# crisbodnar/text-to-image

Hardware: AMD Instinct MI355X
Metric: images/sec (G+D step) at 64x64 batch=64 (higher is better)
Workload: dtype f32; 1 GPU; wgancls 64x64 batch=64/GPU fp32, synthetic images + random 1024-d text embeddings, D step (+kt) then G step, Adam(b1=0,b2=0.9); global_batch=64, parallelism=dp1, launch=hipGraph replay (1 graph/iteration)

## Files before the change

### text-to-image_amd/csrc/t2i_bgemm.hip

```cpp
#include <hip/hip_runtime.h>
#include <stdint.h>

#include <type_traits>

#include "t2i_internal.h"

namespace t2i {

typedef float f32x16 __attribute__((ext_vector_type(16)));
typedef unsigned int u32x4 __attribute__((ext_vector_type(4)));

namespace {
constexpr int BK = 32;
constexpr int KSTRIDE = BK + 4;
constexpr unsigned OOB = 0xFFFFFFF0u;

template <int LAY, int WM, int WN, int NW = 4>
struct BSmem {
  static constexpr bool A_KIN = LAY != 2, B_KIN = LAY == 1;
  static constexpr int BM = 32 * (NW / 2) * WM, BN = 64 * WN;
  static constexpr int A_ELEMS = A_KIN ? BM * KSTRIDE : BK * BM;
  static constexpr int B_ELEMS = B_KIN ? BN * KSTRIDE : BK * BN;
  static constexpr int BYTES = 2 * (A_ELEMS + B_ELEMS) * 4;
};
// ... 29 lines not shown
  const int n_items = (runlen - slot + nslot - 1) / nslot;
  const int tiles = p.tiles_m * p.tiles_n;

  auto coords = [&](int w, int& bz, int& bm, int& bn) __attribute__((always_inline)) {
    bz = w / tiles;
    const int t = w - bz * tiles;
    const int g = p.group_n, per_group = g * p.tiles_m;
    const int grp = t / per_group, rr = t - grp * per_group, n0 = grp * g;
    const int width = min(g, p.tiles_n - n0);
    const int tm = rr / width;
    bm = tm * BM;
    bn = (n0 + rr - tm * width) * BN;
  };

  const int kq = tid & 7, r0 = tid >> 3;
  const int a_c4 = tid % A_C4, a_kr = tid / A_C4, b_c4 = tid % B_C4, b_kr = tid / B_C4;
  __amdgpu_buffer_rsrc_t ra, rb;
  int a_off[A_LD], b_off[B_LD];
  bool a_ok[A_LD], b_ok[B_LD];
  int l_item = -1, l_t = 0;

  auto next_item = [&]() __attribute__((always_inline)) {
    ++l_item;
    l_t = 0;
    if (l_item >= n_items) {
#pragma unroll
      for (int i = 0; i < A_LD; ++i) a_ok[i] = false;
#pragma unroll
      for (int i = 0; i < B_LD; ++i) b_ok[i] = false;
      return;
    }
    int bz, bm, bn;
    coords(run0 + slot + l_item * nslot, bz, bm, bn);
    ra = __builtin_amdgcn_make_buffer_rsrc(const_cast<float*>(p.a + (int64_t)bz * p.sa), (short)0, (int)p.a_bytes, 0x00020000);
    rb = __builtin_amdgcn_make_buffer_rsrc(const_cast<float*>(p.b + (int64_t)bz * p.sb), (short)0, (int)p.b_bytes, 0x00020000);
#pragma unroll
    for (int i = 0; i < A_LD; ++i) {
      if (A_KIN) {
        const int m = bm + r0 + RPP * i;
        a_ok[i] = m < p.M;
        a_off[i] = m * p.K + kq * 4;
      } else {
        const int m = bm + a_c4 * 4;
        a_ok[i] = m < p.M;
        a_off[i] = (a_kr + A_KR * i) * p.M + m;
      }
    }
#pragma unroll
    for (int i = 0; i < B_LD; ++i) {
      if (B_KIN) {
        const int n = bn + r0 + RPP * i;
        b_ok[i] = n < p.N;
        b_off[i] = n * p.K + kq * 4;
      } else {
        const int n = bn + b_c4 * 4;
        b_ok[i] = n < p.N;
        b_off[i] = (b_kr + B_KR * i) * p.N + n;
      }
    }
  };

  float4 areg[A_LD], breg[B_LD];
  auto load_into = [&](float4* ar, float4* br) __attribute__((always_inline)) {
    const int k0 = l_t * BK;
    ++l_t;
#pragma unroll
    for (int i = 0; i < A_LD; ++i) {
      if (A_KIN) ar[i] = bl4(ra, a_off[i] + k0, a_ok[i] & (k0 + kq * 4 < p.K));
// ... 674 lines not shown
```

### text-to-image_amd/csrc/t2i_capi.hip

```cpp
#include <hip/hip_runtime.h>
#include <atomic>
#include <initializer_list>
#include <stdarg.h>
#include <stdio.h>
#include <stdlib.h>
#include <string.h>

#include "t2i_internal.h"

namespace t2i {

static thread_local char g_err[512] = "";

void set_error(const char* fmt, ...) {
  va_list ap;
  va_start(ap, fmt);
  vsnprintf(g_err, sizeof(g_err), fmt, ap);
  va_end(ap);
}

size_t col_reduce_ws(int64_t rows, int C);
hipError_t col_reduce_launch(const void*, const void*, const float*, int64_t, int, float*, float*, int, void*, hipStream_t, bool in_bf16 = false);
hipError_t bn_stats_launch(const void*, int64_t, int, float*, float*, const float*, const float*, float, float, float*, float*, float*,
                           float*, float*, float*, void*, hipStream_t, bool x_bf16 = false);
// ... 165 lines not shown
    v.bgemm = env_int("T2I_BGEMM", 1);
    v.bgemm_tile = env_int("T2I_BGEMM_TILE", 0);
    v.bgemm_big_items = env_int("T2I_BGEMM_BIG_ITEMS", 2048);
    v.dma_ovh = env_int("T2I_DMA_OVH", 120);
    v.dma_split_us = env_int("T2I_DMA_SPLIT_US", 29);
    v.tile8_eff = env_int("T2I_TILE8_EFF", 0);
    v.colred_wgs = env_int("T2I_COLRED_WGS", 768);
    v.wino_fuse = env_int("T2I_WINO_FUSE", 1);
    v.wino_fuse_items = env_int("T2I_WINO_FUSE_ITEMS", 512);
    v.wino_fuse_xf = env_int("T2I_WINO_FUSE_XF", 1);
    v.bn_fuse = env_int("T2I_BN_FUSE", 1);
    v.colred_cap = env_int("T2I_COLRED_CAP", 192);
    v.bf16_waves = env_int("T2I_BF16_WAVES", 8);
    v.bf16_pair_tiles = env_int("T2I_BF16_PAIR_TILES", 0);
    v.pair_reduce = env_int("T2I_PAIR_REDUCE", 1);
    v.h_stats = env_int("T2I_H_STATS", 0);
    v.pair_cus = env_int("T2I_PAIR_CUS", 128);
    v.pair_max_px = env_int("T2I_PAIR_MAX_PX", 49152);
    v.pair = env_int("T2I_PAIR", 1);
    v.vec_epi = env_int("T2I_VEC_EPI", 1);
    v.batch_lin = env_int("T2I_BATCH_LIN", 1);
    v.no_ut = env_int("T2I_NO_UT", 0);
    v.no_thin = env_int("T2I_NO_THIN", 0);
    v.winograd = env_int("T2I_WINOGRAD", 1);
    v.winograd_minc = env_int("T2I_WINOGRAD_MINC", 128);
    v.winograd_maxhw = env_int("T2I_WINOGRAD_MAXHW", 1024);
    v.winograd_minwork = env_int("T2I_WINOGRAD_MINWORK", 50000000);
    v.winograd_k4s2 = env_int("T2I_WINOGRAD_K4S2", 1);
    v.winograd_k4s2_minc = env_int("T2I_WINOGRAD_K4S2_MINC", 128);
    v.winograd_k4s2_bwd_minc = env_int("T2I_WINOGRAD_K4S2_BWD_MINC", 128);
    v.winograd_k4s2_bwdf = env_int("T2I_WINOGRAD_K4S2_BWDF", 1);
    v.winograd_k4s2_minwork = env_int("T2I_WINOGRAD_K4S2_MINWORK", 160000000);
    v.winograd_k4s2_minitems = env_int("T2I_WINOGRAD_K4S2_MINITEMS", 400);
    v.adam_blocks = env_int("T2I_ADAM_BLOCKS", 2048);
    v.cache_refresh = env_int("T2I_CACHE_REFRESH", 0);
    v.thin_parts = env_int("T2I_THIN_PARTS", 2);
    v.bf16_operands = env_int("T2I_BF16_OPERANDS", 1);
    v.max_chain = env_int("T2I_MAX_CHAIN", 8192);
    const char* sc = getenv("T2I_SPLIT_COST");
    v.split_cost = (sc && *sc) ? atof(sc) : 4.0;
    return v;
  }();
  return t;
}

const Tuning& tuning() { return tuning_mut(); }

static Plan make_plan(int64_t M, int64_t N, int64_t K, int nphase, size_t out_elems, int split_cap = 32, int math = 0, bool batched = false,
                      int bk = 32, int m_unit = 0,
                      bool dma = false,
                      int cus = 256) {
  static const int cand[5][2] = {{2, 2}, {2, 1}, {1, 2}, {1, 1}, {4, 2}};
  static const double rel_eff_f32[4] = {1.0, 0.93, 0.93, 0.94};
  static const double rel_eff_bf16[4] = {1.0, 0.74, 0.74, 0.55};
  static const int max_resident_f32[4] = {2, 3, 3, 4};
  static const int max_resident_bf16[4] = {3, 4, 4, 4};
  static const double share_eff_f32[5] = {0.0, 0.80, 0.95, 1.0, 1.0};
  static const double share_eff_bf16[5] = {0.0, 0.62, 0.86, 1.0, 1.0};
  const double rel_eff_dma[5] = {1.0, 0.82, 0.83, 0.64, tuning().tile8_eff * 0.01};
  static const int max_resident_dma[5] = {3, 3, 3, 6, 1};
  static const double share_eff_dma[7] = {0.0, 0.75, 1.0, 1.0, 1.0, 1.0, 1.0};
  const bool hft = math && m_unit > 0 && (m_unit % 128) == 0 && tuning().bf16_dma;
  const double hft_boost = hft ? tuning().hft_boost * 0.01 : 1.0;
  const double* rel_eff = dma ? rel_eff_dma : (math ? rel_eff_bf16 : rel_eff_f32);
  const int* max_resident = dma ? max_resident_dma : (math ? max_resident_bf16 : max_resident_f32);
  const double* share_eff = dma ? share_eff_dma : (math ? share_eff_bf16 : share_eff_f32);
// ... 287 lines not shown
    if (tuning().debug_plan) fprintf(stderr, "[t2i stage] cast_bf16 x (filter gradient): B=%d %dx%dx%d->%d k%d s%d\n", d->B, d->H, d->W, d->Cin, d->Cout, d->KH, d->SH);
    rc = check(cast_bf16_launch(x, nx, base, stream), what);
    if (rc != T2I_OK) return rc;
    x_h = base;
  }
  if (!dy_h || !aligned16(dy_h)) {
    if (tuning().debug_plan) fprintf(stderr, "[t2i stage] cast_bf16 dy (filter gradient): B=%d %dx%dx%d->%d k%d s%d\n", d->B, d->H, d->W, d->Cin, d->Cout, d->KH, d->SH);
    rc = check(cast_bf16_launch(dy, ny, base + off_y, stream), what);
    if (rc != T2I_OK) return rc;
    dy_h = base + off_y;
  }
  p.a = reinterpret_cast<const float*>(x_h); p.b = reinterpret_cast<const float*>(dy_h);
  p.a_bytes = (uint32_t)(nx * 2); p.b_bytes = (uint32_t)(ny * 2);
  p.tiles_m = pl.tiles_m; p.tiles_n = pl.tiles_n; p.group_n = 1;
  p.splitk = pl.splitk; p.k_per_split = pl.k_per_split;
  p.out_elems = out_elems;
  p.bias = nullptr; p.act = T2I_ACT_NONE; p.alpha = 0.f;
  if (pl.splitk > 1) { p.c = reinterpret_cast<float*>(base + off_s); p.accumulate = 0; }
  else { p.c = dw; p.accumulate = accumulate; }
  if (defer) {
    defer->set = true; defer->mode = MODE_BWD_FILTER; defer->wmt = pl.wmt; defer->wnt = pl.wnt; defer->p = p;
    defer->slabs = reinterpret_cast<const float*>(base + off_s); defer->bias = nullptr; defer->act = T2I_ACT_NONE; defer->alpha = 0.f; defer->out = dw;
    defer->accumulate = accumulate; defer->out_h = nullptr; defer->out_h_written = nullptr;
    return T2I_OK;
  }
  rc = check(igemm_h_filter_launch(p, pl.wmt, pl.wnt, stream), what);
  if (rc != T2I_OK) return rc;
  if (pl.splitk > 1)
    rc = check(splitk_reduce_launch(reinterpret_cast<const float*>(base + off_s), pl.splitk, out_elems, nullptr, p.N, T2I_ACT_NONE, 0.f, dw,
                                    accumulate, stream), what);
  return rc;
}

int run_batched_gemm(const t2i_conv_desc& gd, int gmode, int nbatch, const float* a, const float* b, float* c, int64_t sa, int64_t sb,
                     int64_t sc, hipStream_t stream, const char* what) {
  {
    const int M = gmode == MODE_BWD_FILTER ? gd.Cin : gd.B;
    const int N = gmode == MODE_BWD_DATA ? gd.Cin : gd.Cout;
    const int K = gmode == MODE_BWD_FILTER ? gd.B : (gmode == MODE_BWD_DATA ? gd.Cout : gd.Cin);
    const int ntiles = (K + 31) / 32;
    const int64_t a_elems = (int64_t)gd.B * (gmode == MODE_BWD_DATA ? gd.Cout : gd.Cin);
    const int64_t b_elems = gmode == MODE_BWD_FILTER ? (int64_t)gd.B * gd.Cout : (int64_t)gd.Cin * gd.Cout;
    if (tuning().bgemm && gd.math != T2I_MATH_BF16 && !tuning().force_tile && (ntiles & 1) == 0 && M % 4 == 0 && N % 4 == 0 && K % 4 == 0 &&
        aligned16(a) && aligned16(b) && sa % 4 == 0 && sb % 4 == 0 && a_elems < (1LL << 30) && b_elems < (1LL << 30)) {
      BgemmParams q;
      memset(&q, 0, sizeof(q));
      q.a = a; q.b = b; q.c = c;
      q.M = M; q.N = N; q.K = K;
      int wm = 1, wn = 1;
      {
        auto items_of = [&](int a_, int b_) { return (int64_t)nbatch * ((M + 64 * a_ - 1) / (64 * a_)) * ((N + 64 * b_ - 1) / (64 * b_)); };
        const int ft = tuning().bgemm_tile;
        const int64_t big = tuning().bgemm_big_items;
        if (ft == 22 || ft == 21 || ft == 12 || ft == 11) { wm = ft / 10; wn = ft % 10; }
        else if (ft == 41 && M >= 128) { wm = 4; wn = 1; }
        else if (M >= 128 && N >= 128 && items_of(2, 2) >= big) { wm = 2; wn = 2; }
        else if (M >= 128 && items_of(2, 1) >= big) { wm = 2; wn = 1; }
        else if (N >= 128 && items_of(1, 2) >= big) { wm = 1; wn = 2; }
      }
      const int bm_rows = wm == 4 ? 128 : 64 * wm;
      q.tiles_m = (M + bm_rows - 1) / bm_rows; q.tiles_n = (N + 64 * wn - 1) / (64 * wn);
      { const int g = tuning().group_n; q.group_n = q.tiles_n < g ? q.tiles_n : g; if (q.group_n < 1) q.group_n = 1; }
      q.ntiles = ntiles;
      const int64_t items = (int64_t)nbatch * q.tiles_m * q.tiles_n;
      if (items < (1LL << 30)) {
        q.items = (int32_t)items;
        q.sa = sa; q.sb = sb; q.sc = sc;
        q.a_bytes = (uint32_t)(a_elems * 4); q.b_bytes = (uint32_t)(b_elems * 4);
        if (tuning().debug_plan)
          fprintf(stderr, "[t2i plan] batched x%d M=%d N=%d K=%d mode %d -> persistent %dx%d, %lld items\n", nbatch, M, N, K, gmode, bm_rows, 64 * wn, (long long)items);
        return check(bgemm_launch(gmode == MODE_FWD ? 0 : (gmode == MODE_BWD_DATA ? 1 : 2), wm, wn, q, stream), what);
      }
    }
  }
  IgemmParams p;
  fill_common(p, &gd);
  p.a = a; p.b = b;
  if (gmode == MODE_BWD_FILTER) {
    p.a_bytes = (uint32_t)((size_t)gd.B * gd.Cin * 4);
    p.b_bytes = (uint32_t)((size_t)gd.B * gd.Cout * 4);
    p.M = gd.Cin; p.N = gd.Cout; p.K = gd.B;
    p.div_c.set(gd.Cin);
    p.walk_db = 32; p.walk_doh = 0;
    p.nbatch = nbatch; p.batch_a = sa; p.batch_b = sb; p.batch_c = sc; p.batch_lin = tuning().batch_lin;
    Plan pl = make_plan(p.M, p.N, p.K, nbatch, (size_t)p.M * p.N, 1, gd.math, true);
    p.tiles_m = pl.tiles_m; p.tiles_n = pl.tiles_n;
    { const int g = tuning().group_n; p.group_n = pl.tiles_n < g ? pl.tiles_n : g; if (p.group_n < 1) p.group_n = 1; }
    p.splitk = 1; p.k_per_split = pl.k_per_split;
    p.out_elems = (size_t)p.M * p.N;
    p.c = c; p.bias = nullptr; p.act = T2I_ACT_NONE; p.alpha = 0.f; p.accumulate = 0;
    const bool vec = (gd.Cin % 4 == 0) && (gd.Cout % 4 == 0) && aligned16(a) && aligned16(b);
    return check(igemm_launch(MODE_BWD_FILTER, p, pl.wmt, pl.wnt, vec ? 2 : 0, stream), what);
  }
  const bool bwd = gmode == MODE_BWD_DATA;
  const int K = bwd ? gd.Cout : gd.Cin, N = bwd ? gd.Cin : gd.Cout;
  p.a_bytes = (uint32_t)((size_t)gd.B * K * 4);
  p.b_bytes = (uint32_t)((size_t)gd.Cin * gd.Cout * 4);
  p.M = gd.B; p.N = N; p.K = K;
  if (bwd) {
    const int kmax = fill_phases(p);
    p.K = kmax;
    p.div_c.set(gd.Cout);
  } else {
    p.div_c.set(gd.Cin);
  }
  p.nbatch = nbatch; p.batch_a = sa; p.batch_b = sb; p.batch_c = sc; p.batch_lin = tuning().batch_lin;
  Plan pl = make_plan(p.M, p.N, p.K, nbatch, (size_t)p.M * p.N, 1, gd.math, true);
// ... 1151 lines not shown
  if (!w || !g || !v || !slot_end_dev || !slot_mult_dev) { set_error("t2i_adam_tf_slots: bad argument (w, g, v or a slot table is NULL)"); return T2I_ERR_INVALID; }
  if (n <= 0 || (n & 3)) { set_error("t2i_adam_tf_slots: n = %lld must be a positive multiple of 4", (long long)n); return T2I_ERR_INVALID; }
  if (n_slots < 1 || n_slots > T2I_ADAM_MAX_SLOTS) {
    set_error("t2i_adam_tf_slots: n_slots = %d is outside [1, %d]", (int)n_slots, (int)T2I_ADAM_MAX_SLOTS);
    return T2I_ERR_INVALID;
  }
  if (!adam_args_ok(a, ADAM_MOMENT | ADAM_ALIGNED)) return T2I_ERR_INVALID;
  if (reinterpret_cast<uintptr_t>(slot_end_dev) & 7) { set_error("t2i_adam_tf_slots: slot_end_dev must be 8-byte aligned"); return T2I_ERR_INVALID; }
  if (!adam_args_ok(a, ADAM_APART)) return T2I_ERR_INVALID;
  for (const float* o : {(const float*)w, g, (const float*)m, (const float*)v, (const float*)ema})
    if (ranges_overlap(slot_end_dev, (uintptr_t)n_slots * 8, o, (uintptr_t)n * 4) || ranges_overlap(slot_mult_dev, (uintptr_t)n_slots * 8, o, (uintptr_t)n * 4)) {
      set_error("t2i_adam_tf_slots: a slot table overlaps an arena");
      return T2I_ERR_INVALID;
    }
  if (!adam_args_ok(a, ADAM_DECAY)) return T2I_ERR_INVALID;
  return adam_update(a, slot_end_dev, slot_mult_dev, (int)n_slots, lr_t, lr_t_dev, beta2, eps, grad_scale, stream);
}

long long t2i_stat(const char* key) {
  if (key && !strcmp(key, "pair_fused")) return g_stat_pair_fused.load();
  return -1;
}

int t2i_tuning_set(const char* key, double value) {
  if (!key) { set_error("t2i_tuning_set: null key"); return T2I_ERR_INVALID; }
  Tuning& t = tuning_mut();
  struct { const char* name; int* field; } ints[] = {
      {"force_tile", &t.force_tile}, {"force_splitk", &t.force_splitk}, {"debug_plan", &t.debug_plan}, {"group_n", &t.group_n},
      {"no_ut", &t.no_ut}, {"no_thin", &t.no_thin}, {"winograd", &t.winograd}, {"winograd_minc", &t.winograd_minc},
      {"winograd_maxhw", &t.winograd_maxhw}, {"winograd_k4s2", &t.winograd_k4s2}, {"winograd_k4s2_minc", &t.winograd_k4s2_minc},
      {"winograd_k4s2_bwd_minc", &t.winograd_k4s2_bwd_minc}, {"winograd_k4s2_bwdf", &t.winograd_k4s2_bwdf}, {"winograd_k4s2_minwork", &t.winograd_k4s2_minwork}, {"winograd_k4s2_minitems", &t.winograd_k4s2_minitems},
      {"adam_blocks", &t.adam_blocks}, {"max_chain", &t.max_chain}, {"bf16_operands", &t.bf16_operands},
      {"cache_refresh", &t.cache_refresh}, {"thin_parts", &t.thin_parts}, {"batch_lin", &t.batch_lin}, {"bgemm", &t.bgemm}, {"winograd_minwork", &t.winograd_minwork}, {"bf16_dma", &t.bf16_dma}, {"hft_boost", &t.hft_boost}, {"hft_ovh", &t.hft_ovh},
      {"bgemm_tile", &t.bgemm_tile}, {"bgemm_big_items", &t.bgemm_big_items}, {"vec_epi", &t.vec_epi}, {"pair", &t.pair}, {"pair_cus", &t.pair_cus}, {"h_stats", &t.h_stats}, {"pair_reduce", &t.pair_reduce}, {"bf16_waves", &t.bf16_waves}, {"bf16_pair_tiles", &t.bf16_pair_tiles}, {"colred_wgs", &t.colred_wgs}, {"colred_cap", &t.colred_cap}, {"bn_fuse", &t.bn_fuse}, {"wino_fuse", &t.wino_fuse}, {"wino_fuse_items", &t.wino_fuse_items}, {"wino_fuse_xf", &t.wino_fuse_xf}, {"tile8_eff", &t.tile8_eff}, {"dma_ovh", &t.dma_ovh}, {"dma_split_us", &t.dma_split_us}, {"pair_max_px", &t.pair_max_px}};
  for (auto& e : ints)
    if (!strcmp(key, e.name)) { *e.field = (int)value; return T2I_OK; }
  if (!strcmp(key, "split_cost")) { t.split_cost = value; return T2I_OK; }
  set_error("t2i_tuning_set: unknown key '%s'", key);
  return T2I_ERR_INVALID;
}

int t2i_kt_sgd(float* kt, const float* wdist_sums, float scale, float lr, t2i_stream_t stream) {
  if (!kt || !wdist_sums) { set_error("t2i_kt_sgd: bad argument"); return T2I_ERR_INVALID; }
  return check(kt_sgd_launch(kt, wdist_sums, scale, lr, (hipStream_t)stream), "t2i_kt_sgd");
}

int t2i_zero_ranges(float* base, const int64_t* ranges, int32_t n, t2i_stream_t stream) {
  if (!base || !ranges || n <= 0) { set_error("t2i_zero_ranges: bad argument"); return T2I_ERR_INVALID; }
  return check(zero_ranges_launch(base, reinterpret_cast<const long long*>(ranges), n, (hipStream_t)stream), "t2i_zero_ranges");
}

int t2i_trunc_normal(float* out, int64_t n, uint64_t seed, uint64_t offset, float mean, float std, float lo, float hi, t2i_stream_t stream) {
  if (!out || n <= 0 || !(std > 0.f) || !(lo < hi)) { set_error("t2i_trunc_normal: bad argument (n > 0, std > 0, lo < hi)"); return T2I_ERR_INVALID; }
  return check(trunc_normal_launch(out, (size_t)n, seed, offset, mean, std, lo, hi, (hipStream_t)stream), "t2i_trunc_normal");
}

int t2i_conv2d_algo(const t2i_conv_desc* d, int32_t which) {
  if (validate_desc(d) || which < 0 || which > 2) return -1;
  const bool thin = !tuning().no_thin;
  if (which == 0) {
    if (thin && (head_conv_eligible(*d) || tiny_conv_eligible(*d, false) || stem_fwd_eligible(*d))) return T2I_ALGO_DIRECT_SMALL;
    if (h_eligible(*d, false)) return T2I_ALGO_IMPLICIT_GEMM_BF16_OPERANDS;
    if (winograd_eligible(*d, false)) return T2I_ALGO_WINOGRAD_F2X2_3X3;
    if (winograd_k4s2_eligible(*d, false)) return T2I_ALGO_WINOGRAD_F2X2_2X2;
  } else if (which == 1) {
    if (thin && (head_conv_eligible(*d) || tiny_conv_eligible(*d, true) || thin_deconv_eligible(*d))) return T2I_ALGO_DIRECT_SMALL;
    if (h_eligible(*d, true)) return T2I_ALGO_IMPLICIT_GEMM_BF16_OPERANDS;
// ... 365 lines not shown
```

### text-to-image_amd/csrc/t2i_internal.h

```cpp
#ifndef T2I_INTERNAL_H
#define T2I_INTERNAL_H

#include <hip/hip_runtime.h>
#include <stddef.h>
#include <stdint.h>

#include "../../include/t2i_hip.h"

namespace t2i {

enum { MODE_FWD = 0, MODE_BWD_DATA = 1, MODE_BWD_FILTER = 2 };

struct FastDiv {
  uint32_t mul, shr, add;
  __host__ void set(uint32_t d) {
    if (d == 1) { mul = 0; shr = 0; add = 0xFFFFFFFFu; return; }
    add = 0;
    uint32_t l = 0;
    while ((1u << l) < d) ++l;
    uint64_t pw = 1ull << (31 + l);
    mul = (uint32_t)((pw + d - 1) / d);
    shr = l - 1;
  }
  __host__ __device__ __forceinline__ int div(int n) const {
// ... 60 lines not shown
    const unsigned long long p0 = (unsigned long long)0xD2511F53u * c0, p1 = (unsigned long long)0xCD9E8D57u * c2;
    const unsigned n0 = (unsigned)(p1 >> 32) ^ c1 ^ k0, n1 = (unsigned)p1, n2 = (unsigned)(p0 >> 32) ^ c3 ^ k1, n3 = (unsigned)p0;
    c0 = n0; c1 = n1; c2 = n2; c3 = n3;
    k0 += 0x9E3779B9u; k1 += 0xBB67AE85u;
  }
  out[0] = c0; out[1] = c1; out[2] = c2; out[3] = c3;
}

bool winograd_eligible(const t2i_conv_desc& d, bool bwd_data);
bool winograd_filter_eligible(const t2i_conv_desc& d);
size_t winograd_ws(const t2i_conv_desc& d, bool bwd_data);
int winograd_conv(const t2i_conv_desc& d, bool bwd_data, const float* in, const float* w, const float* bias, float* out, int act,
                  float alpha, void* ws, size_t ws_bytes, hipStream_t stream, float* Vkeep = nullptr);
bool winograd_k4s2_eligible(const t2i_conv_desc& d, bool bwd_data);
size_t winograd_k4s2_filter_grad_ws(const t2i_conv_desc& d);
int winograd_k4s2_filter_grad(const t2i_conv_desc& d, const float* x, const float* dy, float* dw, int accumulate, void* ws, size_t ws_bytes,
                              hipStream_t stream, const float* Vhave = nullptr, int valid_rows = 0x7fffffff);
int filter_cache_enable(int on);
int filter_cache_attach(void* buf, size_t bytes);
void filter_cache_invalidate(const void* p, size_t bytes);
size_t filter_cache_bytes();
int filter_cache_refresh(const void* p, size_t bytes, hipStream_t stream);
int filter_cache_assume(const void* p, size_t bytes, hipStream_t stream);
size_t winograd_k4s2_bwd_ws(const t2i_conv_desc& d);
int winograd_k4s2_bwd_data(const t2i_conv_desc& d, const float* dy, const float* w, const float* bias, float* dx, int act, float alpha,
                           void* ws, size_t ws_bytes, hipStream_t stream);
size_t winograd_k4s2_ws(const t2i_conv_desc& d);
int winograd_k4s2_fwd(const t2i_conv_desc& d, const float* x, const float* w, const float* bias, float* y, int act, float alpha, void* ws,
                      size_t ws_bytes, hipStream_t stream, float* Vkeep = nullptr);
size_t winograd_filter_grad_ws(const t2i_conv_desc& d);
int winograd_filter_grad(const t2i_conv_desc& d, const float* x, const float* dy, float* dw, int accumulate, void* ws, size_t ws_bytes,
                         hipStream_t stream, const float* Vhave = nullptr, int valid_rows = 0x7fffffff, int plane_rows = 0);
int run_batched_gemm(const t2i_conv_desc& gd, int gmode, int nbatch, const float* a, const float* b, float* c, int64_t sa, int64_t sb, int64_t sc,
                     hipStream_t stream, const char* what);

hipError_t igemm_launch(int mode, const IgemmParams& p, int wmt, int wnt, int var, hipStream_t stream);
hipError_t igemm_h_launch(int mode, const IgemmParams& p, int wmt, int wnt, hipStream_t stream);
hipError_t igemm_h_filter_launch(const IgemmParams& p, int wmt, int wnt, hipStream_t stream);
bool igemm_pair_fusable(const IgemmParams& pb, int wmt_b, int wnt_b);
hipError_t igemm_pair_launch(int mode, const IgemmParams& pa, int wmt, int wnt, const IgemmParams& pb, hipStream_t stream);
hipError_t cast_bf16_launch(const float* x, size_t n, void* y, hipStream_t stream);
hipError_t cast_bf16_any_launch(const float* x, size_t n, void* y, hipStream_t stream);
hipError_t cast_f32_launch(const void* x_bf16, size_t n, float* y, hipStream_t stream);
hipError_t wcast_launch(const float* w, int taps, int Ci, int Co, int transpose, void* out, hipStream_t stream);
float* filter_cache_get(const float* w, int kind, int Cin, int Cout, size_t bytes, hipStream_t stream, bool* fill);
struct ReduceJob {
  const float* slabs; const float* bias; float* out; void* out_h; size_t out_elems; float alpha; int splitk, N, act, accumulate, blocks;
};
bool splitk_reduce2_ok(const ReduceJob& a, const ReduceJob& b);
hipError_t splitk_reduce2_launch(ReduceJob a, ReduceJob b, hipStream_t stream);
hipError_t splitk_reduce_launch(const float* slabs, int splitk, size_t out_elems, const float* bias, int N, int act,
                                float alpha, float* out, int accumulate, hipStream_t stream, void* out_h = nullptr, bool* wrote_h = nullptr);

void set_error(const char* fmt, ...);

struct BgemmParams {
  const float* a;
  const float* b;
  float* c;
  int32_t M, N, K;
  int32_t tiles_m, tiles_n, group_n;
  int32_t ntiles;
  int32_t items;
  int64_t sa, sb, sc;
  uint32_t a_bytes, b_bytes;
};
hipError_t bgemm_launch(int lay, int wm, int wn, const BgemmParams& p, hipStream_t stream);
struct Bgemm9Params {
  BgemmParams g;
  const float* bias;
  float* out;
  int32_t OH, OW, Th, Tw;
  int32_t sr;
  int32_t act;
  float alpha;
  const float* dy;
  int32_t dHo, dWo;
};
hipError_t bgemm9_launch(int lay, const Bgemm9Params& q, hipStream_t stream);

struct Tuning {
  int force_tile, force_splitk, debug_plan, group_n, no_ut, no_thin;
  int winograd, winograd_minc, winograd_maxhw, winograd_k4s2, winograd_k4s2_minc, winograd_k4s2_bwd_minc, winograd_k4s2_bwdf;
  int adam_blocks, max_chain, bf16_operands, cache_refresh, thin_parts, batch_lin, bgemm, winograd_minwork, bf16_dma, hft_boost, hft_ovh, bgemm_tile, bgemm_big_items, vec_epi, pair, pair_cus, pair_max_px, dma_ovh, dma_split_us, tile8_eff, colred_wgs, colred_cap, h_stats, pair_reduce, bf16_waves, bf16_pair_tiles, bn_fuse, wino_fuse, wino_fuse_items, wino_fuse_xf, winograd_k4s2_minwork, winograd_k4s2_minitems;
  double split_cost;
};
const Tuning& tuning();

}
#endif
```

### text-to-image_amd/csrc/t2i_winograd.hip

```cpp
#include <hip/hip_runtime.h>
#include <stdint.h>
#include <stdio.h>
#include <string.h>
#include <stdlib.h>

#include <mutex>
#include <vector>

#include "t2i_internal.h"

namespace t2i {

struct FilterEntry {
  const float* w; int kind, Cin, Cout; float* U; size_t bytes; unsigned long long cap; hipStream_t stream; bool valid;
  hipStream_t cap_fill = nullptr;
};
static std::mutex g_fc_mu;
static std::vector<FilterEntry> g_fc;
static int g_fc_on = 0;
static char* g_fc_buf = nullptr;
static size_t g_fc_cap = 0, g_fc_used = 0;

int filter_cache_attach(void* buf, size_t bytes) {
  std::lock_guard<std::mutex> lk(g_fc_mu);
// ... 178 lines not shown
      const float4 m0 = m[(size_t)wino_slot(0, c, flip) * plane], m1 = m[(size_t)wino_slot(1, c, flip) * plane],
                   m2 = m[(size_t)wino_slot(2, c, flip) * plane], m3 = m[(size_t)wino_slot(3, c, flip) * plane];
      z[0][c] = f4add(f4add(m0, m1), m2);
      z[1][c] = f4sub(f4sub(m1, m2), m3);
    }
    const float4 bs = bias ? reinterpret_cast<const float4*>(bias)[n4] : make_float4(0.f, 0.f, 0.f, 0.f);
#pragma unroll
    for (int r = 0; r < 2; ++r) {
      float4 y0 = f4add(f4add(f4add(z[r][0], z[r][1]), z[r][2]), bs);
      float4 y1 = f4add(f4sub(f4sub(z[r][1], z[r][2]), z[r][3]), bs);
      y0.x = apply_act(y0.x, act, alpha); y0.y = apply_act(y0.y, act, alpha); y0.z = apply_act(y0.z, act, alpha); y0.w = apply_act(y0.w, act, alpha);
      y1.x = apply_act(y1.x, act, alpha); y1.y = apply_act(y1.y, act, alpha); y1.z = apply_act(y1.z, act, alpha); y1.w = apply_act(y1.w, act, alpha);
      float4* o = reinterpret_cast<float4*>(y + ((b * H + 2 * ty + r) * W + 2 * tx) * N) + n4;
      o[0] = y0;
      o[N4] = y1;
    }
  }
}

static int wino_min_channels() { return tuning().winograd_minc; }

bool winograd_eligible(const t2i_conv_desc& d, bool bwd_data) {
  if (!tuning().winograd || d.math != T2I_MATH_F32) return false;
  if (!(d.KH == 3 && d.KW == 3 && d.SH == 1 && d.SW == 1 && d.pad_t == 1 && d.pad_l == 1 && d.Ho == d.H && d.Wo == d.W)) return false;
  if ((d.H & 1) || (d.W & 1) || (d.Cin % 32) || (d.Cout % 32)) return false;
  const int cmin = d.Cin < d.Cout ? d.Cin : d.Cout;
  const int maxhw = tuning().winograd_maxhw;
  if (cmin < wino_min_channels() || (int64_t)d.H * d.W > maxhw) return false;
  const int64_t T = (int64_t)d.B * (d.H / 2) * (d.W / 2);
  return T * d.Cin * d.Cout >= (int64_t)tuning().winograd_minwork;
}

bool winograd_filter_eligible(const t2i_conv_desc& d) {
  return winograd_eligible(d, false) && (int64_t)d.Cin * d.Cout >= 65536;
}

static void wino_dims(const t2i_conv_desc& d, bool bwd, size_t* T, int* K, int* N) {
  *T = (size_t)d.B * (d.H / 2) * (d.W / 2);
  *K = bwd ? d.Cout : d.Cin;
  *N = bwd ? d.Cin : d.Cout;
}

size_t winograd_ws(const t2i_conv_desc& d, bool bwd) {
  size_t T; int K, N;
  wino_dims(d, bwd, &T, &K, &N);
  return al256((size_t)16 * K * N * 4) + al256(16 * T * K * 4) + al256(16 * T * N * 4);
}

int winograd_conv(const t2i_conv_desc& d, bool bwd, const float* in, const float* w, const float* bias, float* out, int act,
                  float alpha, void* ws, size_t ws_bytes, hipStream_t stream, float* Vkeep) {
  size_t T; int K, N;
  wino_dims(d, bwd, &T, &K, &N);
  if (!ws || ws_bytes < winograd_ws(d, bwd) || (reinterpret_cast<uintptr_t>(ws) & 15)) {
    set_error("winograd conv: workspace %zu B < %zu B required (or misaligned)", ws_bytes, winograd_ws(d, bwd));
    return T2I_ERR_WORKSPACE;
  }
  char* base = reinterpret_cast<char*>(ws);
  float* U = reinterpret_cast<float*>(base);
  float* V = Vkeep ? Vkeep : reinterpret_cast<float*>(base + al256((size_t)16 * K * N * 4));
  float* Mx = reinterpret_cast<float*>(base + al256((size_t)16 * K * N * 4) + al256(16 * T * K * 4));
  const int Th = d.H / 2, Tw = d.W / 2;
  bool fill = true;
  if (float* Uc = filter_cache_get(w, 0, d.Cin, d.Cout, (size_t)16 * K * N * 4, stream, &fill)) U = Uc;
  if (fill)
    hipLaunchKernelGGL(wino_filter_kernel, dim3(wino_blocks((size_t)K * N)), dim3(256), 0, stream, w, d.Cin, d.Cout, U);
  hipLaunchKernelGGL(wino_input_kernel, dim3(wino_blocks(T * (K / 4))), dim3(256), 0, stream, in, d.H, d.W, K, Th, Tw, T, V, bwd ? 1 : 0, T);
  t2i_conv_desc gd = d;
// ... 4 lines not shown
                     bwd ? 1 : 0);
  const hipError_t e = hipGetLastError();
  if (e != hipSuccess) { set_error("winograd conv: %s", hipGetErrorString(e)); return T2I_ERR_LAUNCH; }
  return T2I_OK;
}

__global__ __launch_bounds__(256) void wino_dy_kernel(const float* __restrict__ dy, int H, int W, int N, int Th, int Tw, size_t T,
                                                      float* __restrict__ Z) {
  const int N4 = N >> 2;
  const size_t total = T * N4, plane = T * N4;
  for (size_t i = (size_t)blockIdx.x * blockDim.x + threadIdx.x; i < total; i += (size_t)gridDim.x * blockDim.x) {
    const int n4 = (int)(i % N4);
    const size_t t = i / N4;
    const int tx = (int)(t % Tw);
    const int ty = (int)((t / Tw) % Th);
    const size_t b = t / ((size_t)Tw * Th);
    const float4* src = reinterpret_cast<const float4*>(dy + ((b * H + 2 * ty) * W + 2 * tx) * N) + n4;
    const float4 d00 = src[0], d01 = src[N4], d10 = src[(size_t)W * N4], d11 = src[(size_t)W * N4 + N4];
    const float4 zero = make_float4(0.f, 0.f, 0.f, 0.f);
    const float4 s[4][2] = {{d00, d01}, {f4add(d00, d10), f4add(d01, d11)}, {f4sub(d00, d10), f4sub(d01, d11)}, {f4sub(zero, d10), f4sub(zero, d11)}};
    float4* o = reinterpret_cast<float4*>(Z) + t * N4 + n4;
#pragma unroll
    for (int r = 0; r < 4; ++r) {
      wst(&o[(size_t)(r * 4 + 0) * plane], s[r][0]);
      wst(&o[(size_t)(r * 4 + 1) * plane], f4add(s[r][0], s[r][1]));
      wst(&o[(size_t)(r * 4 + 2) * plane], f4sub(s[r][0], s[r][1]));
      wst(&o[(size_t)(r * 4 + 3) * plane], f4sub(zero, s[r][1]));
    }
  }
}

__device__ __forceinline__ float4 f4half(float4 a) { return make_float4(0.5f * a.x, 0.5f * a.y, 0.5f * a.z, 0.5f * a.w); }

__global__ __launch_bounds__(256) void wino_dw_kernel(const float* __restrict__ P, int Cin, int Cout, int accumulate,
                                                      float* __restrict__ dw) {
  const int N4 = Cout >> 2;
  const size_t total = (size_t)Cin * N4, plane = total;
  for (size_t i = (size_t)blockIdx.x * blockDim.x + threadIdx.x; i < total; i += (size_t)gridDim.x * blockDim.x) {
    const float4* p = reinterpret_cast<const float4*>(P) + i;
    float4 q[3][4];
#pragma unroll
    for (int c = 0; c < 4; ++c) {
      const float4 p0 = p[(size_t)(0 * 4 + c) * plane], p1 = p[(size_t)(1 * 4 + c) * plane], p2 = p[(size_t)(2 * 4 + c) * plane],
                   p3 = p[(size_t)(3 * 4 + c) * plane];
      const float4 hs = f4half(f4add(p1, p2)), hd = f4half(f4sub(p1, p2));
      q[0][c] = f4add(p0, hs);
      q[1][c] = hd;
      q[2][c] = f4add(hs, p3);
    }
    float4* o = reinterpret_cast<float4*>(dw) + i;
#pragma unroll
    for (int r = 0; r < 3; ++r) {
      const float4 hs = f4half(f4add(q[r][1], q[r][2])), hd = f4half(f4sub(q[r][1], q[r][2]));
      float4 w0 = f4add(q[r][0], hs), w1 = hd, w2 = f4add(hs, q[r][3]);
      if (accumulate) {
        w0 = f4add(w0, o[(size_t)(r * 3 + 0) * plane]); w1 = f4add(w1, o[(size_t)(r * 3 + 1) * plane]); w2 = f4add(w2, o[(size_t)(r * 3 + 2) * plane]);
      }
      wst(&o[(size_t)(r * 3 + 0) * plane], w0);
      wst(&o[(size_t)(r * 3 + 1) * plane], w1);
      wst(&o[(size_t)(r * 3 + 2) * plane], w2);
    }
  }
}

size_t winograd_filter_grad_ws(const t2i_conv_desc& d) {
  const size_t T = (size_t)d.B * (d.H / 2) * (d.W / 2);
  return al256(16 * T * d.Cin * 4) + al256(16 * T * d.Cout * 4) + al256((size_t)16 * d.Cin * d.Cout * 4);
}

int winograd_filter_grad(const t2i_conv_desc& d, const float* x, const float* dy, float* dw, int accumulate, void* ws, size_t ws_bytes,
                         hipStream_t stream, const float* Vhave, int valid_rows, int plane_rows) {
  const size_t T = (size_t)d.B * (d.H / 2) * (d.W / 2);
  const size_t Tp = (Vhave && plane_rows > d.B) ? (size_t)plane_rows * (d.H / 2) * (d.W / 2) : T;
  if (!ws || ws_bytes < winograd_filter_grad_ws(d) || (reinterpret_cast<uintptr_t>(ws) & 15)) {
    set_error("winograd filter gradient: workspace %zu B < %zu B required (or misaligned)", ws_bytes, winograd_filter_grad_ws(d));
    return T2I_ERR_WORKSPACE;
  }
  char* base = reinterpret_cast<char*>(ws);
  float* V = reinterpret_cast<float*>(base);
  float* Z = reinterpret_cast<float*>(base + al256(16 * T * d.Cin * 4));
  float* P = reinterpret_cast<float*>(base + al256(16 * T * d.Cin * 4) + al256(16 * T * d.Cout * 4));
  const int Th = d.H / 2, Tw = d.W / 2;
  if (Vhave) {
    V = const_cast<float*>(Vhave);
    if (valid_rows < d.B) {
      const size_t t0 = (size_t)valid_rows * Th * Tw, Tr = T - t0;
      hipLaunchKernelGGL(wino_input_kernel, dim3(wino_blocks(Tr * (d.Cin / 4))), dim3(256), 0, stream, x + (size_t)valid_rows * d.H * d.W * d.Cin, d.H,
                         d.W, d.Cin, Th, Tw, Tr, V + t0 * d.Cin, 0, Tp);
    }
  } else hipLaunchKernelGGL(wino_input_kernel, dim3(wino_blocks(T * (d.Cin / 4))), dim3(256), 0, stream, x, d.H, d.W, d.Cin, Th, Tw, T, V, 0, T);
  hipLaunchKernelGGL(wino_dy_kernel, dim3(wino_blocks(T * (d.Cout / 4))), dim3(256), 0, stream, dy, d.H, d.W, d.Cout, Th, Tw, T, Z);
  t2i_conv_desc gd = d;
  gd.B = (int32_t)T; gd.H = gd.W = gd.Ho = gd.Wo = 1; gd.KH = gd.KW = gd.SH = gd.SW = 1; gd.pad_t = gd.pad_l = 0;
  const int rc = run_batched_gemm(gd, MODE_BWD_FILTER, 16, V, Z, P, (int64_t)Tp * d.Cin, (int64_t)T * d.Cout, (int64_t)d.Cin * d.Cout, stream,
                                  "winograd filter-gradient gemm");
  if (rc != T2I_OK) return rc;
  hipLaunchKernelGGL(wino_dw_kernel, dim3(wino_blocks((size_t)d.Cin * (d.Cout / 4))), dim3(256), 0, stream, P, d.Cin, d.Cout, accumulate, dw);
  const hipError_t e = hipGetLastError();
  if (e != hipSuccess) { set_error("winograd filter gradient: %s", hipGetErrorString(e)); return T2I_ERR_LAUNCH; }
  return T2I_OK;
}

__device__ __forceinline__ void wino2_filter_body(const float* __restrict__ w, int Cin, int Cout, float* __restrict__ U, unsigned vb, unsigned nvb) {
  const int N4 = Cout >> 2;
  const size_t total = (size_t)4 * Cin * N4;
  const size_t plane = (size_t)4 * Cin * N4;
  for (size_t i = (size_t)vb * 256 + threadIdx.x; i < total; i += (size_t)nvb * 256) {
    const int n4 = (int)(i % N4);
    const int ci = (int)((i / N4) % Cin);
    const int ph = (int)(i / ((size_t)N4 * Cin));
    const int p = ph >> 1, q = ph & 1;
    float4 g[2][2];
#pragma unroll
    for (int a = 0; a < 2; ++a)
#pragma unroll
      for (int b = 0; b < 2; ++b)
        g[a][b] = reinterpret_cast<const float4*>(w + ((size_t)((2 * a + p) * 4 + (2 * b + q)) * Cin + ci) * Cout)[n4];
    float4 s[3][2] = {{g[0][0], g[0][1]}, {f4add(g[0][0], g[1][0]), f4add(g[0][1], g[1][1])}, {g[1][0], g[1][1]}};
    float4* o = reinterpret_cast<float4*>(U) + ((size_t)ph * Cin + ci) * N4 + n4;
#pragma unroll
    for (int r = 0; r < 3; ++r) {
      wst(&o[(size_t)(r * 3 + 0) * plane], s[r][0]);
      wst(&o[(size_t)(r * 3 + 1) * plane], f4add(s[r][0], s[r][1]));
      wst(&o[(size_t)(r * 3 + 2) * plane], s[r][1]);
    }
  }
}

__global__ __launch_bounds__(256) void wino2_filter_kernel(const float* __restrict__ w, int Cin, int Cout, float* __restrict__ U) {
  wino2_filter_body(w, Cin, Cout, U, blockIdx.x, gridDim.x);
// ... 585 lines not shown
```

### text-to-image_amd/stacked.py

```python
import torch
from torch.autograd import Function

from . import autograd as A
from . import kernels as K

_FIRST = [0]


class first_order_pass(object):

    def __init__(self, rows):
        self.rows = int(rows)

    def __enter__(self):
        self.prev, _FIRST[0] = _FIRST[0], self.rows

    def __exit__(self, *a):
        _FIRST[0] = self.prev


class Stacked(object):
    __slots__ = ('main', 'hat')

    def __init__(self, main, hat):
# ... 129 lines not shown
        gh = K.rebatch(ctx.geom4, gp4.shape[0] - R)
        rec = ctx.defer
        if rec is None or rec['done'] or A._INPUTS_ONLY[0] or torch.is_grad_enabled():
            g_dy, g_w, _ = A.bwd_data_backward(gp4[R:], w, None, ggh, gh, K.ACT_NONE, 0.0, False, None,
                                               (ctx.needs_input_grad[1], ctx.needs_input_grad[2], False))
            return None, g_dy, g_w, None, None, None
        g_dy = A.Conv2dFn.apply(ggh, w, None, gh, K.ACT_NONE, 0.0, False, gp4.dtype) if ctx.needs_input_grad[1] else None
        x4, d4 = rec['x4'], ctx.geom4[0]
        tang = _c(ggh)
        if tang.data_ptr() != x4[R:].data_ptr():
            K.axpby(tang, 1.0, out=x4[R:])
        K._drop_image(x4)
        xf, sink, ws4 = rec['xform'], rec['sink'], ctx.geom4[1]
        acc = A.sink_accumulate(w.data_ptr())
        launch = lambda: K.conv_bwd_filter(x4, gp4, d4, ws4, out=sink, xform=xf, xform_valid_rows=R if xf is not None else 0, accumulate=acc)
        A.sunk_launch(launch, (x4, gp4, xf))
        A._notify(w)
        rec['done'] = True
        rec['x4'] = rec['gp4'] = rec['xform'] = None
        return None, g_dy, None, None, None, None


class SConv2dFn(Function):

    @staticmethod
    def forward(ctx, xm, xh, w, b, geom4, act, alpha, want_stats=False):
        R = xm.shape[0]
        x4 = full(xm, xh)
        d, ws = geom4
        assert d.B == x4.shape[0], (d.B, tuple(x4.shape))
        ctx.set_materialize_grads(False)
        ctx.geom_b4 = K.bwd_geom(geom4)
        keep = bool(ctx.needs_input_grad[2]) and not A._INPUTS_ONLY[0] and ctx.geom_b4 is geom4 and (
            (bool(ctx.needs_input_grad[0]) and _DEFER[0]) or not ctx.needs_input_grad[1])
        y4 = (K.conv_fwd_stats if want_stats else K.conv_fwd)(x4, w, b, d, ws, act, alpha, keep_xform=keep)
        ctx.xform = K.LAST_XFORM[0] if keep else None
        K.LAST_XFORM[0] = None
        ctx.save_for_backward(x4, w, y4 if act != K.ACT_NONE else None)
        ctx.R, ctx.act, ctx.alpha, ctx.has_bias, ctx.bias_ref = R, act, alpha, b is not None, b
        return y4[:R], y4[R:]

    @staticmethod
    def backward(ctx, gym, gyh):
        if gym is None and gyh is None:
            return (None,) * 8
        x4, w, y4 = ctx.saved_tensors
        R, B4 = ctx.R, x4.shape[0]
        need_xm, need_xh, need_w, need_b = ctx.needs_input_grad[:4]
        geo_m, geo_h = K.rebatch(ctx.geom_b4, R), K.rebatch(ctx.geom_b4, B4 - R)
        if not _both(gym, gyh):
            gxm = gxh = gw = gb = None
            for g, sl, geom, nx in ((gym, slice(0, R), geo_m, need_xm), (gyh, slice(R, B4), geo_h, need_xh)):
                if g is None:
                    continue
                xf = ctx.xform if sl.start == 0 else None
                gx, gw1, gb1 = A.conv2d_backward(x4[sl], w, y4[sl] if y4 is not None else None, g, geom, ctx.act, ctx.alpha,
                                                 ctx.has_bias, ctx.bias_ref, (nx, need_w, need_b), xf, B4 if xf is not None else 0)
                if sl.start == 0:
                    gxm = gx
                else:
                    gxh = gx
                gw = gw1 if gw is None else (gw if gw1 is None else gw + gw1)
                gb = gb1 if gb is None else (gb if gb1 is None else gb + gb1)
            ctx.xform = None
            return gxm, gxh, gw, gb, None, None, None, None
        bsink = A.sink_at(ctx.bias_ref.data_ptr()) if (ctx.has_bias and need_b) else None
        fuse_b = bsink is not None and ctx.act != K.ACT_NONE and gym.shape[-1] % 4 == 0
# ... 258 lines not shown
```

Before: 5249 images/sec.

## Split Winograd filter-gradient GEMM K into tile slabs and widen eligibility

The Winograd filter-gradient batched GEMM can now split its long reduction dimension (the tile count T) into several slabs. Each slab becomes its own batch member with its own buffer bounds, and the final transform kernel sums the slab partials before applying the output transform. This gives more parallel work items when Cin*Cout is small, and lets layers with small channel products but many tiles take the Winograd path. The cost is a larger workspace and extra partial-sum reads in the transform kernel. The Python side also keeps the forward transform only when the layer has nonzero transform bytes.

```diff
diff --git a/text-to-image_amd/csrc/t2i_bgemm.hip b/text-to-image_amd/csrc/t2i_bgemm.hip
--- a/text-to-image_amd/csrc/t2i_bgemm.hip
+++ b/text-to-image_amd/csrc/t2i_bgemm.hip
@@ -85,8 +85,17 @@
     }
     int bz, bm, bn;
     coords(run0 + slot + l_item * nslot, bz, bm, bn);
-    ra = __builtin_amdgcn_make_buffer_rsrc(const_cast<float*>(p.a + (int64_t)bz * p.sa), (short)0, (int)p.a_bytes, 0x00020000);
-    rb = __builtin_amdgcn_make_buffer_rsrc(const_cast<float*>(p.b + (int64_t)bz * p.sb), (short)0, (int)p.b_bytes, 0x00020000);
+    if (LAY == 2 && p.nslab > 1) {
+      const int pl = bz / p.nslab, sl = bz - pl * p.nslab;
+      const bool last = sl == p.nslab - 1;
+      ra = __builtin_amdgcn_make_buffer_rsrc(const_cast<float*>(p.a + (int64_t)pl * p.sa + (int64_t)sl * p.sa_slab), (short)0,
+                                             (int)(last ? p.a_bytes_last : p.a_bytes), 0x00020000);
+      rb = __builtin_amdgcn_make_buffer_rsrc(const_cast<float*>(p.b + (int64_t)pl * p.sb + (int64_t)sl * p.sb_slab), (short)0,
+                                             (int)(last ? p.b_bytes_last : p.b_bytes), 0x00020000);
+    } else {
+      ra = __builtin_amdgcn_make_buffer_rsrc(const_cast<float*>(p.a + (int64_t)bz * p.sa), (short)0, (int)p.a_bytes, 0x00020000);
+      rb = __builtin_amdgcn_make_buffer_rsrc(const_cast<float*>(p.b + (int64_t)bz * p.sb), (short)0, (int)p.b_bytes, 0x00020000);
+    }
 #pragma unroll
     for (int i = 0; i < A_LD; ++i) {
       if (A_KIN) {
diff --git a/text-to-image_amd/csrc/t2i_capi.hip b/text-to-image_amd/csrc/t2i_capi.hip
--- a/text-to-image_amd/csrc/t2i_capi.hip
+++ b/text-to-image_amd/csrc/t2i_capi.hip
@@ -221,6 +221,8 @@
     v.winograd_k4s2_bwdf = env_int("T2I_WINOGRAD_K4S2_BWDF", 1);
     v.winograd_k4s2_minwork = env_int("T2I_WINOGRAD_K4S2_MINWORK", 160000000);
     v.winograd_k4s2_minitems = env_int("T2I_WINOGRAD_K4S2_MINITEMS", 400);
+    v.wino3_slabs = env_int("T2I_WINO3_SLABS", 0);
+    v.wino3_filter_mint = env_int("T2I_WINO3_FILTER_MINT", 32768);
     v.adam_blocks = env_int("T2I_ADAM_BLOCKS", 2048);
     v.cache_refresh = env_int("T2I_CACHE_REFRESH", 0);
     v.thin_parts = env_int("T2I_THIN_PARTS", 2);
@@ -574,8 +576,14 @@
   return rc;
 }
 
+bool batched_gemm_slabs_ok() { return tuning().bgemm && !tuning().force_tile; }
+
 int run_batched_gemm(const t2i_conv_desc& gd, int gmode, int nbatch, const float* a, const float* b, float* c, int64_t sa, int64_t sb,
-                     int64_t sc, hipStream_t stream, const char* what) {
+                     int64_t sc, hipStream_t stream, const char* what, int nslab, int64_t sa_slab, int64_t sb_slab, int k_last) {
+  if (nslab > 1 && (gmode != MODE_BWD_FILTER || nbatch % nslab || k_last < 1 || k_last > gd.B)) {
+    set_error("%s: K slabs are the filter gradient's (planes x slabs members, 1 <= k_last <= K)", what);
+    return T2I_ERR_INVALID;
+  }
   {
     const int M = gmode == MODE_BWD_FILTER ? gd.Cin : gd.B;
     const int N = gmode == MODE_BWD_DATA ? gd.Cin : gd.Cout;
@@ -609,12 +617,18 @@
         q.items = (int32_t)items;
         q.sa = sa; q.sb = sb; q.sc = sc;
         q.a_bytes = (uint32_t)(a_elems * 4); q.b_bytes = (uint32_t)(b_elems * 4);
+        q.nslab = 1;
+        if (nslab > 1) {
+          q.nslab = nslab; q.sa_slab = sa_slab; q.sb_slab = sb_slab;
+          q.a_bytes_last = (uint32_t)((int64_t)k_last * gd.Cin * 4); q.b_bytes_last = (uint32_t)((int64_t)k_last * gd.Cout * 4);
+        }
         if (tuning().debug_plan)
           fprintf(stderr, "[t2i plan] batched x%d M=%d N=%d K=%d mode %d -> persistent %dx%d, %lld items\n", nbatch, M, N, K, gmode, bm_rows, 64 * wn, (long long)items);
         return check(bgemm_launch(gmode == MODE_FWD ? 0 : (gmode == MODE_BWD_DATA ? 1 : 2), wm, wn, q, stream), what);
       }
     }
   }
+  if (nslab > 1) { set_error("%s: K slabs need the persistent batched GEMM", what); return T2I_ERR_INVALID; }
   IgemmParams p;
   fill_common(p, &gd);
   p.a = a; p.b = b;
@@ -1832,7 +1846,8 @@
       {"winograd_k4s2_bwd_minc", &t.winograd_k4s2_bwd_minc}, {"winograd_k4s2_bwdf", &t.winograd_k4s2_bwdf}, {"winograd_k4s2_minwork", &t.winograd_k4s2_minwork}, {"winograd_k4s2_minitems", &t.winograd_k4s2_minitems},
       {"adam_blocks", &t.adam_blocks}, {"max_chain", &t.max_chain}, {"bf16_operands", &t.bf16_operands},
       {"cache_refresh", &t.cache_refresh}, {"thin_parts", &t.thin_parts}, {"batch_lin", &t.batch_lin}, {"bgemm", &t.bgemm}, {"winograd_minwork", &t.winograd_minwork}, {"bf16_dma", &t.bf16_dma}, {"hft_boost", &t.hft_boost}, {"hft_ovh", &t.hft_ovh},
-      {"bgemm_tile", &t.bgemm_tile}, {"bgemm_big_items", &t.bgemm_big_items}, {"vec_epi", &t.vec_epi}, {"pair", &t.pair}, {"pair_cus", &t.pair_cus}, {"h_stats", &t.h_stats}, {"pair_reduce", &t.pair_reduce}, {"bf16_waves", &t.bf16_waves}, {"bf16_pair_tiles", &t.bf16_pair_tiles}, {"colred_wgs", &t.colred_wgs}, {"colred_cap", &t.colred_cap}, {"bn_fuse", &t.bn_fuse}, {"wino_fuse", &t.wino_fuse}, {"wino_fuse_items", &t.wino_fuse_items}, {"wino_fuse_xf", &t.wino_fuse_xf}, {"tile8_eff", &t.tile8_eff}, {"dma_ovh", &t.dma_ovh}, {"dma_split_us", &t.dma_split_us}, {"pair_max_px", &t.pair_max_px}};
+      {"bgemm_tile", &t.bgemm_tile}, {"bgemm_big_items", &t.bgemm_big_items}, {"vec_epi", &t.vec_epi}, {"pair", &t.pair}, {"pair_cus", &t.pair_cus}, {"h_stats", &t.h_stats}, {"pair_reduce", &t.pair_reduce}, {"bf16_waves", &t.bf16_waves}, {"bf16_pair_tiles", &t.bf16_pair_tiles}, {"colred_wgs", &t.colred_wgs}, {"colred_cap", &t.colred_cap}, {"bn_fuse", &t.bn_fuse}, {"wino_fuse", &t.wino_fuse}, {"wino_fuse_items", &t.wino_fuse_items}, {"wino_fuse_xf", &t.wino_fuse_xf}, {"tile8_eff", &t.tile8_eff}, {"dma_ovh", &t.dma_ovh}, {"dma_split_us", &t.dma_split_us}, {"pair_max_px", &t.pair_max_px},
+      {"wino3_slabs", &t.wino3_slabs}, {"wino3_filter_mint", &t.wino3_filter_mint}};
   for (auto& e : ints)
     if (!strcmp(key, e.name)) { *e.field = (int)value; return T2I_OK; }
   if (!strcmp(key, "split_cost")) { t.split_cost = value; return T2I_OK; }
diff --git a/text-to-image_amd/csrc/t2i_internal.h b/text-to-image_amd/csrc/t2i_internal.h
--- a/text-to-image_amd/csrc/t2i_internal.h
+++ b/text-to-image_amd/csrc/t2i_internal.h
@@ -116,7 +116,8 @@
 int winograd_filter_grad(const t2i_conv_desc& d, const float* x, const float* dy, float* dw, int accumulate, void* ws, size_t ws_bytes,
                          hipStream_t stream, const float* Vhave = nullptr, int valid_rows = 0x7fffffff, int plane_rows = 0);
 int run_batched_gemm(const t2i_conv_desc& gd, int gmode, int nbatch, const float* a, const float* b, float* c, int64_t sa, int64_t sb, int64_t sc,
-                     hipStream_t stream, const char* what);
+                     hipStream_t stream, const char* what, int nslab = 1, int64_t sa_slab = 0, int64_t sb_slab = 0, int k_last = 0);
+bool batched_gemm_slabs_ok();
 
 hipError_t igemm_launch(int mode, const IgemmParams& p, int wmt, int wnt, int var, hipStream_t stream);
 hipError_t igemm_h_launch(int mode, const IgemmParams& p, int wmt, int wnt, hipStream_t stream);
@@ -148,6 +149,9 @@
   int32_t items;
   int64_t sa, sb, sc;
   uint32_t a_bytes, b_bytes;
+  int32_t nslab;
+  int64_t sa_slab, sb_slab;
+  uint32_t a_bytes_last, b_bytes_last;
 };
 hipError_t bgemm_launch(int lay, int wm, int wn, const BgemmParams& p, hipStream_t stream);
 struct Bgemm9Params {
@@ -166,7 +170,7 @@
 struct Tuning {
   int force_tile, force_splitk, debug_plan, group_n, no_ut, no_thin;
   int winograd, winograd_minc, winograd_maxhw, winograd_k4s2, winograd_k4s2_minc, winograd_k4s2_bwd_minc, winograd_k4s2_bwdf;
-  int adam_blocks, max_chain, bf16_operands, cache_refresh, thin_parts, batch_lin, bgemm, winograd_minwork, bf16_dma, hft_boost, hft_ovh, bgemm_tile, bgemm_big_items, vec_epi, pair, pair_cus, pair_max_px, dma_ovh, dma_split_us, tile8_eff, colred_wgs, colred_cap, h_stats, pair_reduce, bf16_waves, bf16_pair_tiles, bn_fuse, wino_fuse, wino_fuse_items, wino_fuse_xf, winograd_k4s2_minwork, winograd_k4s2_minitems;
+  int adam_blocks, max_chain, bf16_operands, cache_refresh, thin_parts, batch_lin, bgemm, winograd_minwork, bf16_dma, hft_boost, hft_ovh, bgemm_tile, bgemm_big_items, vec_epi, pair, pair_cus, pair_max_px, dma_ovh, dma_split_us, tile8_eff, colred_wgs, colred_cap, h_stats, pair_reduce, bf16_waves, bf16_pair_tiles, bn_fuse, wino_fuse, wino_fuse_items, wino_fuse_xf, winograd_k4s2_minwork, winograd_k4s2_minitems, wino3_slabs, wino3_filter_mint;
   double split_cost;
 };
 const Tuning& tuning();
diff --git a/text-to-image_amd/csrc/t2i_winograd.hip b/text-to-image_amd/csrc/t2i_winograd.hip
--- a/text-to-image_amd/csrc/t2i_winograd.hip
+++ b/text-to-image_amd/csrc/t2i_winograd.hip
@@ -234,7 +234,10 @@
 }
 
 bool winograd_filter_eligible(const t2i_conv_desc& d) {
-  return winograd_eligible(d, false) && (int64_t)d.Cin * d.Cout >= 65536;
+  if (!winograd_eligible(d, false)) return false;
+  if ((int64_t)d.Cin * d.Cout >= 65536) return true;
+  const int64_t T = (int64_t)d.B * (d.H / 2) * (d.W / 2);
+  return batched_gemm_slabs_ok() && T >= (int64_t)tuning().wino3_filter_mint;
 }
 
 static void wino_dims(const t2i_conv_desc& d, bool bwd, size_t* T, int* K, int* N) {
@@ -305,17 +308,23 @@
 
 __device__ __forceinline__ float4 f4half(float4 a) { return make_float4(0.5f * a.x, 0.5f * a.y, 0.5f * a.z, 0.5f * a.w); }
 
-__global__ __launch_bounds__(256) void wino_dw_kernel(const float* __restrict__ P, int Cin, int Cout, int accumulate,
+__global__ __launch_bounds__(256) void wino_dw_kernel(const float* __restrict__ P, int Cin, int Cout, int nslab, int accumulate,
                                                       float* __restrict__ dw) {
   const int N4 = Cout >> 2;
   const size_t total = (size_t)Cin * N4, plane = total;
   for (size_t i = (size_t)blockIdx.x * blockDim.x + threadIdx.x; i < total; i += (size_t)gridDim.x * blockDim.x) {
     const float4* p = reinterpret_cast<const float4*>(P) + i;
+    float4 m[16];
+#pragma unroll
+    for (int xi = 0; xi < 16; ++xi) m[xi] = p[(size_t)xi * nslab * plane];
+    for (int sl = 1; sl < nslab; ++sl) {
+#pragma unroll
+      for (int xi = 0; xi < 16; ++xi) m[xi] = f4add(m[xi], p[((size_t)xi * nslab + sl) * plane]);
+    }
     float4 q[3][4];
 #pragma unroll
     for (int c = 0; c < 4; ++c) {
-      const float4 p0 = p[(size_t)(0 * 4 + c) * plane], p1 = p[(size_t)(1 * 4 + c) * plane], p2 = p[(size_t)(2 * 4 + c) * plane],
-                   p3 = p[(size_t)(3 * 4 + c) * plane];
+      const float4 p0 = m[0 * 4 + c], p1 = m[1 * 4 + c], p2 = m[2 * 4 + c], p3 = m[3 * 4 + c];
       const float4 hs = f4half(f4add(p1, p2)), hd = f4half(f4sub(p1, p2));
       q[0][c] = f4add(p0, hs);
       q[1][c] = hd;
@@ -336,9 +345,28 @@
   }
 }
 
+static int wino3_slabs(const t2i_conv_desc& d, size_t* chunk) {
+  const size_t T = (size_t)d.B * (d.H / 2) * (d.W / 2);
+  *chunk = T;
+  if (!batched_gemm_slabs_ok()) return 1;
+  const int forced = tuning().wino3_slabs;
+  const int64_t items = (int64_t)16 * ((d.Cin + 63) / 64) * ((d.Cout + 63) / 64);
+  int64_t want = forced > 0 ? forced : 512 / items;
+  if (forced <= 0 && want > (int64_t)(T / 2048)) want = (int64_t)(T / 2048);
+  if (want > 64) want = 64;
+  if (want <= 1) return 1;
+  const size_t c = ((T + want - 1) / want + 63) & ~(size_t)63;
+  const int S = (int)((T + c - 1) / c);
+  if (S <= 1) return 1;
+  *chunk = c;
+  return S;
+}
+
 size_t winograd_filter_grad_ws(const t2i_conv_desc& d) {
   const size_t T = (size_t)d.B * (d.H / 2) * (d.W / 2);
-  return al256(16 * T * d.Cin * 4) + al256(16 * T * d.Cout * 4) + al256((size_t)16 * d.Cin * d.Cout * 4);
+  size_t chunk;
+  const int S = wino3_slabs(d, &chunk);
+  return al256(16 * T * d.Cin * 4) + al256(16 * T * d.Cout * 4) + al256((size_t)16 * S * d.Cin * d.Cout * 4);
 }
 
 int winograd_filter_grad(const t2i_conv_desc& d, const float* x, const float* dy, float* dw, int accumulate, void* ws, size_t ws_bytes,
@@ -363,12 +391,17 @@
     }
   } else hipLaunchKernelGGL(wino_input_kernel, dim3(wino_blocks(T * (d.Cin / 4))), dim3(256), 0, stream, x, d.H, d.W, d.Cin, Th, Tw, T, V, 0, T);
   hipLaunchKernelGGL(wino_dy_kernel, dim3(wino_blocks(T * (d.Cout / 4))), dim3(256), 0, stream, dy, d.H, d.W, d.Cout, Th, Tw, T, Z);
+  size_t chunk;
+  const int S = wino3_slabs(d, &chunk);
   t2i_conv_desc gd = d;
-  gd.B = (int32_t)T; gd.H = gd.W = gd.Ho = gd.Wo = 1; gd.KH = gd.KW = gd.SH = gd.SW = 1; gd.pad_t = gd.pad_l = 0;
-  const int rc = run_batched_gemm(gd, MODE_BWD_FILTER, 16, V, Z, P, (int64_t)Tp * d.Cin, (int64_t)T * d.Cout, (int64_t)d.Cin * d.Cout, stream,
-                                  "winograd filter-gradient gemm");
+  gd.B = (int32_t)chunk; gd.H = gd.W = gd.Ho = gd.Wo = 1; gd.KH = gd.KW = gd.SH = gd.SW = 1; gd.pad_t = gd.pad_l = 0;
+  if (S > 1 && tuning().debug_plan)
+    fprintf(stderr, "[t2i plan] winograd filter gradient: %d tile slabs of %zu (last %zu) of T=%zu, plane stride %zu tiles\n", S, chunk,
+            T - (size_t)(S - 1) * chunk, T, Tp);
+  const int rc = run_batched_gemm(gd, MODE_BWD_FILTER, 16 * S, V, Z, P, (int64_t)Tp * d.Cin, (int64_t)T * d.Cout, (int64_t)d.Cin * d.Cout, stream,
+                                  "winograd filter-gradient gemm", S, (int64_t)chunk * d.Cin, (int64_t)chunk * d.Cout, (int)(T - (size_t)(S - 1) * chunk));
   if (rc != T2I_OK) return rc;
-  hipLaunchKernelGGL(wino_dw_kernel, dim3(wino_blocks((size_t)d.Cin * (d.Cout / 4))), dim3(256), 0, stream, P, d.Cin, d.Cout, accumulate, dw);
+  hipLaunchKernelGGL(wino_dw_kernel, dim3(wino_blocks((size_t)d.Cin * (d.Cout / 4))), dim3(256), 0, stream, P, d.Cin, d.Cout, S, accumulate, dw);
   const hipError_t e = hipGetLastError();
   if (e != hipSuccess) { set_error("winograd filter gradient: %s", hipGetErrorString(e)); return T2I_ERR_LAUNCH; }
   return T2I_OK;
diff --git a/text-to-image_amd/stacked.py b/text-to-image_amd/stacked.py
--- a/text-to-image_amd/stacked.py
+++ b/text-to-image_amd/stacked.py
@@ -185,7 +185,8 @@
         ctx.set_materialize_grads(False)
         ctx.geom_b4 = K.bwd_geom(geom4)
         keep = bool(ctx.needs_input_grad[2]) and not A._INPUTS_ONLY[0] and ctx.geom_b4 is geom4 and (
-            (bool(ctx.needs_input_grad[0]) and _DEFER[0]) or not ctx.needs_input_grad[1])
+            (bool(ctx.needs_input_grad[0]) and _DEFER[0]) or
+            (not ctx.needs_input_grad[1] and K.conv_xform_bytes(K.rebatch(geom4, R)[0]) > 0))
         y4 = (K.conv_fwd_stats if want_stats else K.conv_fwd)(x4, w, b, d, ws, act, alpha, keep_xform=keep)
         ctx.xform = K.LAST_XFORM[0] if keep else None
         K.LAST_XFORM[0] = None
```

After: 5260 images/sec, median of 6. About the same (+0.2%).
